# meta-pytorch/torchft

Measured on AMD Instinct MI355X. Metric: goodput_tokens_per_sec, higher is better.
Workload: dtype bf16; 1 GPU; model=llama3_8b, global_batch=4, seq_len=8192, parallelism=ft-dp1, fault_tolerance=True

## Files before the change

### csrc/kernels/flash_attn_bwd.hip

```cpp

#include <hip/hip_bf16.h>
#include <hip/hip_runtime.h>

#include <cstdint>

namespace torchft_amd {

using bf16 = __hip_bfloat16;
typedef __attribute__((__vector_size__(8 * sizeof(short)))) short bf16x8_vec;
typedef __attribute__((__vector_size__(16 * sizeof(float)))) float f32x16;

#define FA_D 128
#define FA_BLK 32
#define FA_WAVES 8
#define FA_THREADS 512
#define SUBT 1040

struct Tile {
  __align__(16) unsigned char sub[8 * SUBT];
};

struct ImageSet {
  Tile a;
  Tile b;
};

__device__ inline int st_addr(int tt, int row, int byte_in_row) {
  return tt * SUBT + row * 32 + byte_in_row;
}

struct SmemFA {
  ImageSet img[2];
  __align__(16) unsigned char pa[FA_WAVES][32 * 64];
  __align__(16) unsigned char pb[FA_WAVES][32 * 64];
  __align__(16) unsigned char v_ops[FA_WAVES][10 * 64 * 16];
};

struct TileRegs {
  uint4 a, b;
};

__device__ inline TileRegs load_tiles(const bf16* __restrict__ srcA,
                                      const bf16* __restrict__ srcB,
                                      int64_t ld) {
  const int t = threadIdx.x;
  const int64_t off = (int64_t)(t >> 4) * ld + (t & 15) * 8;
  TileRegs r;
  r.a = reinterpret_cast<const uint4*>(srcA + off)[0];
  r.b = reinterpret_cast<const uint4*>(srcB + off)[0];
  return r;
}

__device__ inline void write_tiles(ImageSet* img, const TileRegs& r) {
  const int t = threadIdx.x;
  const int addr = st_addr((t & 15) >> 1, t >> 4, (t & 1) * 16);
  *reinterpret_cast<uint4*>(img->a.sub + addr) = r.a;
  *reinterpret_cast<uint4*>(img->b.sub + addr) = r.b;
}

__device__ inline bf16x8_vec rm_bfrag(const unsigned char* tile, int tt, int half,
                                      int l31) {
  return *reinterpret_cast<const bf16x8_vec*>(tile + st_addr(tt, l31, half * 16));
}

__device__ inline int row_swz(int row, int byte_off) {
  return byte_off ^ ((((row >> 2) ^ (row >> 4)) & 3) << 4);
}
__device__ inline int pb_addr(int row, int byte_off) {
  return row * 64 + row_swz(row, byte_off);
}
__device__ inline bf16x8_vec pb_afrag(const unsigned char* pb, int h2, int half,
                                      int l31) {
  return *reinterpret_cast<const bf16x8_vec*>(pb + pb_addr(l31, h2 * 32 + half * 16));
}
__device__ inline int c_row(int reg, int half) {
  return (reg & 3) + 8 * (reg >> 2) + 4 * half;
}

__device__ inline unsigned tr_lane_off(int lane) {
  return ((lane >> 4) & 1) * SUBT + ((lane >> 5) * 8) * 32 + (lane & 15) * 8;
}

#define TR_READ(dst, addr) \
  asm volatile("ds_read_b64_tr_b16 %0, %1" : "=v"(dst) : "v"(addr))

#define TR_WAIT4_KEEP(N, r0, r1, r2, r3)              \
  asm volatile("s_waitcnt lgkmcnt(" #N ")"            \
               : "+v"(r0), "+v"(r1), "+v"(r2), "+v"(r3))
#define TR_WAIT2_KEEP(N, r0, r1) \
  asm volatile("s_waitcnt lgkmcnt(" #N ")" : "+v"(r0), "+v"(r1))

__device__ inline int64_t row_off(int b, int h, int s, int H, int S, int bshd) {
  return bshd ? (((int64_t)b * S + s) * H + h) * FA_D
              : (((int64_t)b * H + h) * S + s) * FA_D;
}

__device__ inline bf16x8_vec tr_join(unsigned long long lo, unsigned long long hi) {
  union {
    struct {
      unsigned long long lo, hi;
    } u;
    bf16x8_vec v;
  } c;
  c.u.lo = lo;
  c.u.hi = hi;
  return c.v;
}

__global__ __launch_bounds__(FA_THREADS, 1) void fa_bwd_dkdv_kernel(
    const bf16* __restrict__ q, const bf16* __restrict__ k,
    const bf16* __restrict__ v, const bf16* __restrict__ dout,
    const float* __restrict__ lse, const float* __restrict__ delta,
    bf16* __restrict__ dk, bf16* __restrict__ dv, int B, int Hq, int Hkv,
    int S, float scale, int causal, int bshd) {
  __shared__ SmemFA sm;
  const int G = Hq / Hkv;
  const int b = blockIdx.y / Hkv;
  const int hkv = blockIdx.y % Hkv;
  const int wave = threadIdx.x >> 6;
  const int lane = threadIdx.x & 63;
  const int half = lane >> 5;
  const int l31 = lane & 31;
  const int jb = blockIdx.x * FA_WAVES + wave;
  const bool active = jb * FA_BLK < S;
  const int nQ = S / FA_BLK;
  const int i_min = causal ? blockIdx.x * FA_WAVES : 0;
  const int nI = nQ - i_min;
  const int T = G * nI;

  unsigned char* vops = sm.v_ops[wave];
  bf16x8_vec kfrag[6];
  if (active) {
    const int64_t kv_off = row_off(b, hkv, jb * FA_BLK + l31, Hkv, S, bshd);
#pragma unroll
    for (int t = 0; t < 8; t++) {
      const bf16x8_vec kv =
          *reinterpret_cast<const bf16x8_vec*>(k + kv_off + t * 16 + half * 8);
      if (t < 6) {
        kfrag[t] = kv;
      } else {
        *reinterpret_cast<bf16x8_vec*>(vops + ((t + 2) * 64 + lane) * 16) = kv;
      }
      *reinterpret_cast<bf16x8_vec*>(vops + (t * 64 + lane) * 16) =
          *reinterpret_cast<const bf16x8_vec*>(v + kv_off + t * 16 + half * 8);
    }
  }

  f32x16 dk_acc[4] = {};
  f32x16 dv_acc[4] = {};

  const int64_t q_ld = bshd ? (int64_t)Hq * FA_D : FA_D;
  const float* lse_base = lse + ((int64_t)b * Hq + hkv * G) * S;
  const float* delta_base = delta + ((int64_t)b * Hq + hkv * G) * S;

  auto tile_src = [&](int t, const bf16* base) -> const bf16* {
    const int g = t / nI;
    const int i = i_min + t % nI;
    return base + row_off(b, hkv * G + g, i * FA_BLK, Hq, S, bshd);
  };

  const unsigned tr_off = tr_lane_off(lane);

  for (int t = 0; t < T; t++) {
    const int cur = t & 1;
    const int g = t / nI;
    const int i = i_min + t % nI;

    {
      TileRegs r = load_tiles(tile_src(t, q), tile_src(t, dout), q_ld);
      write_tiles(&sm.img[cur], r);
    }
    __syncthreads();

    if (active && !(causal && i < jb)) {
      const ImageSet* img = &sm.img[cur];
      const float lse_q = lse_base[(int64_t)g * S + i * FA_BLK + l31];
      const float delta_q = delta_base[(int64_t)g * S + i * FA_BLK + l31];

      f32x16 s_acc = {};
      f32x16 dp_acc = {};
#pragma unroll
      for (int tt = 0; tt < 8; tt++) {
        const bf16x8_vec vf =
            *reinterpret_cast<const bf16x8_vec*>(vops + (tt * 64 + lane) * 16);
        const bf16x8_vec kf =
            tt < 6 ? kfrag[tt]
                   : *reinterpret_cast<const bf16x8_vec*>(
                         vops + ((tt + 2) * 64 + lane) * 16);
        s_acc = __builtin_amdgcn_mfma_f32_32x32x16_bf16(
            kf, rm_bfrag(img->a.sub, tt, half, l31), s_acc, 0, 0, 0);
        dp_acc = __builtin_amdgcn_mfma_f32_32x32x16_bf16(
            vf, rm_bfrag(img->b.sub, tt, half, l31), dp_acc, 0, 0, 0);
      }

      const int qg = i * FA_BLK + l31;
      unsigned char* pa = sm.pa[wave];
      unsigned char* pb = sm.pb[wave];
#pragma unroll
      for (int rg = 0; rg < 16; rg++) {
        const int row = c_row(rg, half);
        const int kg = jb * FA_BLK + row;
        const bool valid = !causal || (qg >= kg);
        const float pv = valid ? __expf(scale * s_acc[rg] - lse_q) : 0.0f;
        *reinterpret_cast<bf16*>(pa + pb_addr(row, l31 * 2)) = __float2bfloat16(pv);
        *reinterpret_cast<bf16*>(pb + pb_addr(row, l31 * 2)) =
            __float2bfloat16(pv * (dp_acc[rg] - delta_q) * scale);
      }
      const unsigned a_base = (unsigned)(uintptr_t)img->a.sub + tr_off;
      const unsigned b_base = (unsigned)(uintptr_t)img->b.sub + tr_off;
#pragma unroll
      for (int it = 0; it < 8; it++) {
        const int dt = it & 3;
        const int h2 = it >> 2;
        const unsigned base = dt * (2 * SUBT) + h2 * 512;
        unsigned long long fd0, fd1, fq0, fq1;
        TR_READ(fd0, b_base + base);
        TR_READ(fd1, b_base + base + 128);
        TR_READ(fq0, a_base + base);
        TR_READ(fq1, a_base + base + 128);
        TR_WAIT4_KEEP(0, fd0, fd1, fq0, fq1);
        dv_acc[dt] = __builtin_amdgcn_mfma_f32_32x32x16_bf16(
            pb_afrag(pa, h2, half, l31), tr_join(fd0, fd1),
            dv_acc[dt], 0, 0, 0);
        dk_acc[dt] = __builtin_amdgcn_mfma_f32_32x32x16_bf16(
            pb_afrag(pb, h2, half, l31), tr_join(fq0, fq1),
            dk_acc[dt], 0, 0, 0);
      }
    }
    __syncthreads();
  }

  if (!active) return;
#pragma unroll
  for (int dt = 0; dt < 4; dt++) {
#pragma unroll
    for (int rg = 0; rg < 16; rg++) {
      const int key = c_row(rg, half);
      const int64_t row = row_off(b, hkv, jb * FA_BLK + key, Hkv, S, bshd);
      const int d = dt * 32 + l31;
      dk[row + d] = __float2bfloat16(dk_acc[dt][rg]);
      dv[row + d] = __float2bfloat16(dv_acc[dt][rg]);
    }
  }
}

#define SUBT64 2080

struct Tile64 {
  __align__(16) unsigned char sub[8 * SUBT64];
};

struct SmemDq {
  Tile64 k_img[2];
  Tile64 v_img[2];
  __align__(16) unsigned char pb[FA_WAVES][32 * 64];
};

__device__ inline int st64_addr(int tt, int row, int byte_in_row) {
  return tt * SUBT64 + row * 32 + byte_in_row;
}

__device__ inline void write_tiles64(Tile64* kd, Tile64* vd,
                                     const bf16* __restrict__ ksrc,
                                     const bf16* __restrict__ vsrc,
                                     int64_t ld) {
  const int t = threadIdx.x;
  const int r = t >> 3;
  const int c0 = (t & 7) * 2;
  const int64_t off = (int64_t)r * ld + c0 * 8;
  const uint4 k0 = reinterpret_cast<const uint4*>(ksrc + off)[0];
  const uint4 k1 = reinterpret_cast<const uint4*>(ksrc + off)[1];
  const uint4 v0 = reinterpret_cast<const uint4*>(vsrc + off)[0];
  const uint4 v1 = reinterpret_cast<const uint4*>(vsrc + off)[1];
  const int a0 = st64_addr(c0 >> 1, r, (c0 & 1) * 16);
  *reinterpret_cast<uint4*>(kd->sub + a0) = k0;
  *reinterpret_cast<uint4*>(kd->sub + a0 + 16) = k1;
  *reinterpret_cast<uint4*>(vd->sub + a0) = v0;
  *reinterpret_cast<uint4*>(vd->sub + a0 + 16) = v1;
}

__device__ inline bf16x8_vec rm64_bfrag(const unsigned char* tile, int tt,
                                        int row, int half) {
  return *reinterpret_cast<const bf16x8_vec*>(
      tile + st64_addr(tt, row, half * 16));
}

__device__ inline unsigned tr64_lane_off(int lane) {
  return ((lane >> 4) & 1) * SUBT64 + ((lane >> 5) * 8) * 32 + (lane & 15) * 8;
}

__global__ __launch_bounds__(FA_THREADS, 1) void fa_bwd_dq_kernel(
    const bf16* __restrict__ q, const bf16* __restrict__ k,
    const bf16* __restrict__ v, const bf16* __restrict__ dout,
    const float* __restrict__ lse, const float* __restrict__ delta,
    bf16* __restrict__ dq, int B, int Hq, int Hkv, int S, float scale,
    int causal, int bshd) {
  __shared__ SmemDq sm;
  const int G = Hq / Hkv;
  const int b = blockIdx.y / Hq;
  const int hq = blockIdx.y % Hq;
  const int hkv = hq / G;
  const int wave = threadIdx.x >> 6;
  const int lane = threadIdx.x & 63;
  const int half = lane >> 5;
  const int l31 = lane & 31;
  const int ib = blockIdx.x * FA_WAVES + wave;
  const bool active = ib * FA_BLK < S;
  const int nK64 = (S + 63) / 64;
  const int kv_hi = causal ? (blockIdx.x * FA_WAVES + FA_WAVES) * FA_BLK : S;
  const int T = causal ? (min(kv_hi, S) + 63) / 64 : nK64;

  bf16x8_vec qfrag[8], dofrag[8];
  float lse_row[16], delta_row[16];
  if (active) {
    const int64_t q_off = row_off(b, hq, ib * FA_BLK + l31, Hq, S, bshd);
#pragma unroll
    for (int t = 0; t < 8; t++) {
      qfrag[t] = *reinterpret_cast<const bf16x8_vec*>(q + q_off + t * 16 + half * 8);
      dofrag[t] = *reinterpret_cast<const bf16x8_vec*>(dout + q_off + t * 16 + half * 8);
    }
    const float* lse_head = lse + ((int64_t)b * Hq + hq) * S;
    const float* delta_head = delta + ((int64_t)b * Hq + hq) * S;
#pragma unroll
    for (int rg = 0; rg < 16; rg++) {
      const int row = ib * FA_BLK + c_row(rg, half);
      lse_row[rg] = lse_head[row];
      delta_row[rg] = delta_head[row];
    }
  }

  f32x16 dq_acc[4] = {};

  const int64_t kv_ld = bshd ? (int64_t)Hkv * FA_D : FA_D;
  const unsigned tr_off = tr64_lane_off(lane);

  for (int j = 0; j < T; j++) {
    const int cur = j & 1;
    write_tiles64(&sm.k_img[cur], &sm.v_img[cur],
                  k + row_off(b, hkv, j * 64, Hkv, S, bshd),
                  v + row_off(b, hkv, j * 64, Hkv, S, bshd), kv_ld);
    __syncthreads();

    if (active && !(causal && j * 64 > ib * FA_BLK + FA_BLK - 1)) {
      const unsigned char* kimg = sm.k_img[cur].sub;
      const unsigned char* vimg = sm.v_img[cur].sub;
      const unsigned a_base = (unsigned)(uintptr_t)kimg + tr_off;
      unsigned char* pb = sm.pb[wave];

#pragma unroll
      for (int s = 0; s < 2; s++) {
        const int kb0 = j * 64 + s * 32;
        if (causal && kb0 > ib * FA_BLK + FA_BLK - 1) break;

        f32x16 s_acc = {};
        f32x16 dp_acc = {};
#pragma unroll
        for (int tt = 0; tt < 8; tt++) {
          s_acc = __builtin_amdgcn_mfma_f32_32x32x16_bf16(
              qfrag[tt], rm64_bfrag(kimg, tt, s * 32 + l31, half), s_acc, 0, 0,
              0);
          dp_acc = __builtin_amdgcn_mfma_f32_32x32x16_bf16(
              dofrag[tt], rm64_bfrag(vimg, tt, s * 32 + l31, half), dp_acc, 0,
              0, 0);
        }

        const int kg = kb0 + l31;
#pragma unroll
        for (int rg = 0; rg < 16; rg++) {
          const int qg = ib * FA_BLK + c_row(rg, half);
          const bool valid = !causal || (qg >= kg);
          const float p = valid ? __expf(scale * s_acc[rg] - lse_row[rg]) : 0.0f;
          const float ds = p * (dp_acc[rg] - delta_row[rg]) * scale;
          *reinterpret_cast<bf16*>(pb + pb_addr(c_row(rg, half), l31 * 2)) =
              __float2bfloat16(ds);
        }

        bf16x8_vec pbf[2];
#pragma unroll
        for (int h2 = 0; h2 < 2; h2++) pbf[h2] = pb_afrag(pb, h2, half, l31);

        const unsigned s_base = a_base + (s * 32) * 32;
        unsigned long long fk0[2], fk1[2];
        TR_READ(fk0[0], s_base);
        TR_READ(fk1[0], s_base + 128);
#pragma unroll
        for (int it = 0; it < 8; it++) {
          const int dt = it & 3;
          const int h2 = it >> 2;
          const int cur2 = it & 1;
          const int nxt = cur2 ^ 1;
          if (it < 7) {
            const int it2 = it + 1;
            const unsigned nbase =
                (it2 & 3) * (2 * SUBT64) + (it2 >> 2) * 512;
            TR_READ(fk0[nxt], s_base + nbase);
            TR_READ(fk1[nxt], s_base + nbase + 128);
            TR_WAIT2_KEEP(2, fk0[cur2], fk1[cur2]);
          } else {
            TR_WAIT2_KEEP(0, fk0[cur2], fk1[cur2]);
          }
          dq_acc[dt] = __builtin_amdgcn_mfma_f32_32x32x16_bf16(
              pbf[h2], tr_join(fk0[cur2], fk1[cur2]), dq_acc[dt], 0, 0, 0);
        }
      }
    }
    __syncthreads();
  }

  if (!active) return;
#pragma unroll
  for (int dt = 0; dt < 4; dt++) {
#pragma unroll
    for (int rg = 0; rg < 16; rg++) {
      dq[row_off(b, hq, ib * FA_BLK + c_row(rg, half), Hq, S, bshd) + dt * 32 +
         l31] = __float2bfloat16(dq_acc[dt][rg]);
    }
  }
}


__global__ void fa_delta_kernel(const bf16* __restrict__ dout,
                                const bf16* __restrict__ o,
                                float* __restrict__ delta, int64_t rows,
                                int Hq, int S, int bshd) {
  const int64_t row = (int64_t)blockIdx.x * (blockDim.x >> 6) + (threadIdx.x >> 6);
  if (row >= rows) return;
  const int lane = threadIdx.x & 63;
  int64_t didx = row;
  if (bshd) {
    const int h = (int)(row % Hq);
    const int64_t bs = row / Hq;
    const int s = (int)(bs % S);
    const int64_t bb = bs / S;
    didx = (bb * Hq + h) * S + s;
  }
  const __hip_bfloat162 d2 =
      *reinterpret_cast<const __hip_bfloat162*>(dout + row * FA_D + lane * 2);
  const __hip_bfloat162 o2 =
      *reinterpret_cast<const __hip_bfloat162*>(o + row * FA_D + lane * 2);
  float2 df = __bfloat1622float2(d2);
  float2 of = __bfloat1622float2(o2);
  float v = df.x * of.x + df.y * of.y;
#pragma unroll
  for (int off = 32; off > 0; off >>= 1) v += __shfl_down(v, off, 64);
  if (lane == 0) delta[didx] = v;
}

void launch_fa_delta(const void* dout, const void* o, float* delta,
                     int64_t rows, int Hq, int S, bool bshd,
                     hipStream_t stream) {
  const int waves_per_wg = 8;
  const int64_t nwg = (rows + waves_per_wg - 1) / waves_per_wg;
  hipLaunchKernelGGL(fa_delta_kernel, dim3((uint32_t)nwg), dim3(waves_per_wg * 64),
                     0, stream, (const bf16*)dout, (const bf16*)o, delta, rows,
                     Hq, S, bshd ? 1 : 0);
}


void launch_fa_bwd(const void* q, const void* k, const void* v, const void* dout,
                   const float* lse, const float* delta, void* dq, void* dk,
                   void* dv, int B, int Hq, int Hkv, int S, float scale,
                   bool causal, bool bshd, hipStream_t stream) {
  const int nblk = (S + FA_BLK * FA_WAVES - 1) / (FA_BLK * FA_WAVES);
  hipLaunchKernelGGL(fa_bwd_dkdv_kernel, dim3(nblk, B * Hkv), dim3(FA_THREADS), 0,
                     stream, (const bf16*)q, (const bf16*)k, (const bf16*)v,
                     (const bf16*)dout, lse, delta, (bf16*)dk, (bf16*)dv, B, Hq,
                     Hkv, S, scale, causal ? 1 : 0, bshd ? 1 : 0);
  hipLaunchKernelGGL(fa_bwd_dq_kernel, dim3(nblk, B * Hq), dim3(FA_THREADS), 0,
                     stream, (const bf16*)q, (const bf16*)k, (const bf16*)v,
                     (const bf16*)dout, lse, delta, (bf16*)dq, B, Hq, Hkv, S,
                     scale, causal ? 1 : 0, bshd ? 1 : 0);
}

}
```

Baseline: 15140 tokens/s.

## Software-pipeline global tile loads and LDS transpose reads in flash attention backward

Both the dK/dV and dQ backward kernels now prefetch the next Q/dO (or K/V) tile, plus the next LSE/delta values, into registers while the current tile is being computed. The registers are written into the alternate LDS buffer afterwards, so only one barrier per iteration remains instead of a load-then-sync pattern. The dK/dV inner loop also double-buffers its transpose LDS reads and hoists the P/dS fragment loads out of the loop. Causal masks and row addresses are simplified, and dQ blocks are launched in reverse order so the longest causal blocks start first. This raises register pressure, which could hurt occupancy or cause spills.

```diff
diff --git a/csrc/kernels/flash_attn_bwd.hip b/csrc/kernels/flash_attn_bwd.hip
--- a/csrc/kernels/flash_attn_bwd.hip
+++ b/csrc/kernels/flash_attn_bwd.hip
@@ -75,6 +75,9 @@
 }
 __device__ inline int c_row(int reg, int half) {
   return (reg & 3) + 8 * (reg >> 2) + 4 * half;
+}
+__device__ inline int pb_row4_addr(int r4, int half, int l31) {
+  return pb_addr(8 * r4 + 4 * half, l31 * 2);
 }
 
 __device__ inline unsigned tr_lane_off(int lane) {
@@ -161,21 +164,23 @@
 
   const unsigned tr_off = tr_lane_off(lane);
 
+  TileRegs nxt = load_tiles(tile_src(0, q), tile_src(0, dout), q_ld);
+  float lse_n = lse_base[i_min * FA_BLK + l31];
+  float delta_n = delta_base[i_min * FA_BLK + l31];
+  write_tiles(&sm.img[0], nxt);
+  __syncthreads();
+
   for (int t = 0; t < T; t++) {
     const int cur = t & 1;
-    const int g = t / nI;
     const int i = i_min + t % nI;
 
-    {
-      TileRegs r = load_tiles(tile_src(t, q), tile_src(t, dout), q_ld);
-      write_tiles(&sm.img[cur], r);
-    }
-    __syncthreads();
-
-    if (active && !(causal && i < jb)) {
+    const float lse_q = lse_n;
+    const float delta_q = delta_n;
+    const bool more = t + 1 < T;
+    const bool computes = active && !(causal && i < jb);
+
+    if (computes) {
       const ImageSet* img = &sm.img[cur];
-      const float lse_q = lse_base[(int64_t)g * S + i * FA_BLK + l31];
-      const float delta_q = delta_base[(int64_t)g * S + i * FA_BLK + l31];
 
       f32x16 s_acc = {};
       f32x16 dp_acc = {};
@@ -193,40 +198,69 @@
             vf, rm_bfrag(img->b.sub, tt, half, l31), dp_acc, 0, 0, 0);
       }
 
-      const int qg = i * FA_BLK + l31;
       unsigned char* pa = sm.pa[wave];
       unsigned char* pb = sm.pb[wave];
+      const int qk = (i - jb) * FA_BLK + l31 - 4 * half;
 #pragma unroll
       for (int rg = 0; rg < 16; rg++) {
-        const int row = c_row(rg, half);
-        const int kg = jb * FA_BLK + row;
-        const bool valid = !causal || (qg >= kg);
+        const bool valid = !causal || (qk >= c_row(rg, 0));
         const float pv = valid ? __expf(scale * s_acc[rg] - lse_q) : 0.0f;
-        *reinterpret_cast<bf16*>(pa + pb_addr(row, l31 * 2)) = __float2bfloat16(pv);
-        *reinterpret_cast<bf16*>(pb + pb_addr(row, l31 * 2)) =
+        const int wr = pb_row4_addr(rg >> 2, half, l31) + (rg & 3) * 64;
+        *reinterpret_cast<bf16*>(pa + wr) = __float2bfloat16(pv);
+        *reinterpret_cast<bf16*>(pb + wr) =
             __float2bfloat16(pv * (dp_acc[rg] - delta_q) * scale);
       }
+    }
+
+    if (more) {
+      const int64_t st = (int64_t)((t + 1) / nI) * S +
+                         (i_min + (t + 1) % nI) * FA_BLK + l31;
+      nxt = load_tiles(tile_src(t + 1, q), tile_src(t + 1, dout), q_ld);
+      lse_n = lse_base[st];
+      delta_n = delta_base[st];
+    }
+
+    if (computes) {
+      const ImageSet* img = &sm.img[cur];
+      unsigned char* pa = sm.pa[wave];
+      unsigned char* pb = sm.pb[wave];
       const unsigned a_base = (unsigned)(uintptr_t)img->a.sub + tr_off;
       const unsigned b_base = (unsigned)(uintptr_t)img->b.sub + tr_off;
+      bf16x8_vec paf[2], pbf[2];
+#pragma unroll
+      for (int h2 = 0; h2 < 2; h2++) {
+        paf[h2] = pb_afrag(pa, h2, half, l31);
+        pbf[h2] = pb_afrag(pb, h2, half, l31);
+      }
+      unsigned long long fd0[2], fd1[2], fq0[2], fq1[2];
+      TR_READ(fd0[0], b_base);
+      TR_READ(fd1[0], b_base + 128);
+      TR_READ(fq0[0], a_base);
+      TR_READ(fq1[0], a_base + 128);
 #pragma unroll
       for (int it = 0; it < 8; it++) {
         const int dt = it & 3;
         const int h2 = it >> 2;
-        const unsigned base = dt * (2 * SUBT) + h2 * 512;
-        unsigned long long fd0, fd1, fq0, fq1;
-        TR_READ(fd0, b_base + base);
-        TR_READ(fd1, b_base + base + 128);
-        TR_READ(fq0, a_base + base);
-        TR_READ(fq1, a_base + base + 128);
-        TR_WAIT4_KEEP(0, fd0, fd1, fq0, fq1);
+        const int c = it & 1;
+        const int n = c ^ 1;
+        if (it < 7) {
+          const unsigned nbase =
+              ((it + 1) & 3) * (2 * SUBT) + ((it + 1) >> 2) * 512;
+          TR_READ(fd0[n], b_base + nbase);
+          TR_READ(fd1[n], b_base + nbase + 128);
+          TR_READ(fq0[n], a_base + nbase);
+          TR_READ(fq1[n], a_base + nbase + 128);
+          TR_WAIT4_KEEP(4, fd0[c], fd1[c], fq0[c], fq1[c]);
+        } else {
+          TR_WAIT4_KEEP(0, fd0[c], fd1[c], fq0[c], fq1[c]);
+        }
         dv_acc[dt] = __builtin_amdgcn_mfma_f32_32x32x16_bf16(
-            pb_afrag(pa, h2, half, l31), tr_join(fd0, fd1),
-            dv_acc[dt], 0, 0, 0);
+            paf[h2], tr_join(fd0[c], fd1[c]), dv_acc[dt], 0, 0, 0);
         dk_acc[dt] = __builtin_amdgcn_mfma_f32_32x32x16_bf16(
-            pb_afrag(pb, h2, half, l31), tr_join(fq0, fq1),
-            dk_acc[dt], 0, 0, 0);
+            pbf[h2], tr_join(fq0[c], fq1[c]), dk_acc[dt], 0, 0, 0);
       }
     }
+    if (more) write_tiles(&sm.img[cur ^ 1], nxt);
     __syncthreads();
   }
 
@@ -260,23 +294,31 @@
   return tt * SUBT64 + row * 32 + byte_in_row;
 }
 
+struct Tile64Regs {
+  uint4 k0, k1, v0, v1;
+};
+
+__device__ inline Tile64Regs load_tiles64(const bf16* __restrict__ ksrc,
+                                          const bf16* __restrict__ vsrc,
+                                          int64_t ld) {
+  const int t = threadIdx.x;
+  const int64_t off = (int64_t)(t >> 3) * ld + (t & 7) * 16;
+  Tile64Regs r;
+  r.k0 = reinterpret_cast<const uint4*>(ksrc + off)[0];
+  r.k1 = reinterpret_cast<const uint4*>(ksrc + off)[1];
+  r.v0 = reinterpret_cast<const uint4*>(vsrc + off)[0];
+  r.v1 = reinterpret_cast<const uint4*>(vsrc + off)[1];
+  return r;
+}
+
 __device__ inline void write_tiles64(Tile64* kd, Tile64* vd,
-                                     const bf16* __restrict__ ksrc,
-                                     const bf16* __restrict__ vsrc,
-                                     int64_t ld) {
+                                     const Tile64Regs& r) {
   const int t = threadIdx.x;
-  const int r = t >> 3;
-  const int c0 = (t & 7) * 2;
-  const int64_t off = (int64_t)r * ld + c0 * 8;
-  const uint4 k0 = reinterpret_cast<const uint4*>(ksrc + off)[0];
-  const uint4 k1 = reinterpret_cast<const uint4*>(ksrc + off)[1];
-  const uint4 v0 = reinterpret_cast<const uint4*>(vsrc + off)[0];
-  const uint4 v1 = reinterpret_cast<const uint4*>(vsrc + off)[1];
-  const int a0 = st64_addr(c0 >> 1, r, (c0 & 1) * 16);
-  *reinterpret_cast<uint4*>(kd->sub + a0) = k0;
-  *reinterpret_cast<uint4*>(kd->sub + a0 + 16) = k1;
-  *reinterpret_cast<uint4*>(vd->sub + a0) = v0;
-  *reinterpret_cast<uint4*>(vd->sub + a0 + 16) = v1;
+  const int a0 = st64_addr(t & 7, t >> 3, 0);
+  *reinterpret_cast<uint4*>(kd->sub + a0) = r.k0;
+  *reinterpret_cast<uint4*>(kd->sub + a0 + 16) = r.k1;
+  *reinterpret_cast<uint4*>(vd->sub + a0) = r.v0;
+  *reinterpret_cast<uint4*>(vd->sub + a0 + 16) = r.v1;
 }
 
 __device__ inline bf16x8_vec rm64_bfrag(const unsigned char* tile, int tt,
@@ -304,10 +346,11 @@
   const int lane = threadIdx.x & 63;
   const int half = lane >> 5;
   const int l31 = lane & 31;
-  const int ib = blockIdx.x * FA_WAVES + wave;
+  const int bx = causal ? (int)(gridDim.x - 1 - blockIdx.x) : (int)blockIdx.x;
+  const int ib = bx * FA_WAVES + wave;
   const bool active = ib * FA_BLK < S;
   const int nK64 = (S + 63) / 64;
-  const int kv_hi = causal ? (blockIdx.x * FA_WAVES + FA_WAVES) * FA_BLK : S;
+  const int kv_hi = causal ? (bx * FA_WAVES + FA_WAVES) * FA_BLK : S;
   const int T = causal ? (min(kv_hi, S) + 63) / 64 : nK64;
 
   bf16x8_vec qfrag[8], dofrag[8];
@@ -334,12 +377,19 @@
   const int64_t kv_ld = bshd ? (int64_t)Hkv * FA_D : FA_D;
   const unsigned tr_off = tr64_lane_off(lane);
 
+  auto tile_regs = [&](int j) -> Tile64Regs {
+    const int64_t off = row_off(b, hkv, j * 64, Hkv, S, bshd);
+    return load_tiles64(k + off, v + off, kv_ld);
+  };
+
+  Tile64Regs pre = tile_regs(0);
+  write_tiles64(&sm.k_img[0], &sm.v_img[0], pre);
+  __syncthreads();
+
   for (int j = 0; j < T; j++) {
     const int cur = j & 1;
-    write_tiles64(&sm.k_img[cur], &sm.v_img[cur],
-                  k + row_off(b, hkv, j * 64, Hkv, S, bshd),
-                  v + row_off(b, hkv, j * 64, Hkv, S, bshd), kv_ld);
-    __syncthreads();
+    const bool more = j + 1 < T;
+    if (more) pre = tile_regs(j + 1);
 
     if (active && !(causal && j * 64 > ib * FA_BLK + FA_BLK - 1)) {
       const unsigned char* kimg = sm.k_img[cur].sub;
@@ -365,14 +415,14 @@
         }
 
         const int kg = kb0 + l31;
+        const int kq = kg - ib * FA_BLK - 4 * half;
 #pragma unroll
         for (int rg = 0; rg < 16; rg++) {
-          const int qg = ib * FA_BLK + c_row(rg, half);
-          const bool valid = !causal || (qg >= kg);
+          const bool valid = !causal || (c_row(rg, 0) >= kq);
           const float p = valid ? __expf(scale * s_acc[rg] - lse_row[rg]) : 0.0f;
           const float ds = p * (dp_acc[rg] - delta_row[rg]) * scale;
-          *reinterpret_cast<bf16*>(pb + pb_addr(c_row(rg, half), l31 * 2)) =
-              __float2bfloat16(ds);
+          *reinterpret_cast<bf16*>(pb + pb_row4_addr(rg >> 2, half, l31) +
+                                   (rg & 3) * 64) = __float2bfloat16(ds);
         }
 
         bf16x8_vec pbf[2];
@@ -404,6 +454,7 @@
         }
       }
     }
+    if (more) write_tiles64(&sm.k_img[cur ^ 1], &sm.v_img[cur ^ 1], pre);
     __syncthreads();
   }
 
```

Result: faster. 15900 tokens/s (median of 6 runs) (+5.0%).
